# carlosnatalino/optical-rl-gym

Measured on AMD Instinct MI355X. Metric: env-steps/sec RMSA-v0 NSFNET batch 65536, higher is better.
Workload: dtype u64 bitmaps + f64 statistics

## Files before the change

optical_rl_gym_amd/csrc/orl_device_split.h:

```cpp
#pragma once
#include "orl_device_g8.h"

namespace orl {
namespace sp {

#define ORL_PROF_SLOTS 48
#define ORL_PROF_WAVES 16384
#ifdef ORL_TIMING
struct Prof { long long t; unsigned long long acc[ORL_PROF_SLOTS]; };
static __device__ unsigned long long g_prof[ORL_PROF_WAVES * ORL_PROF_SLOTS];
#define ORL_PROF_BEGIN_() do { for (int k_ = 0; k_ < ORL_PROF_SLOTS; k_++) prof.acc[k_] = 0; prof.t = clock64(); } while (0)
#define ORL_PROF_(k) do { long long n_ = clock64(); prof.acc[k] += (unsigned long long)(n_ - prof.t); prof.t = n_; } while (0)
#define ORL_PROF_END_() do { if ((threadIdx.x & 63) == 0) { const size_t w_ = ((size_t)blockIdx.x * (blockDim.x >> 6) + (threadIdx.x >> 6)) % ORL_PROF_WAVES; \
    unsigned long long* g_ = ::orl::sp::g_prof + w_ * ORL_PROF_SLOTS; \
    for (int k_ = 0; k_ < ORL_PROF_SLOTS; k_++) g_[k_] += prof.acc[k_]; } } while (0)
#define ORL_PROF_BEGIN() ORL_PROF_BEGIN_()
#define ORL_PROF_END() ORL_PROF_END_()
#define ORL_PROFA(k) ORL_PROF_(k)
#define ORL_PROF(k) ORL_PROF_(16 + (k))
#define ORL_PROFR(k) ORL_PROF_(32 + (k))
#else
struct Prof { long long t; };
#define ORL_PROF_BEGIN() do { } while (0)
#define ORL_PROF_END() do { } while (0)
// ... 1185 lines not shown
      e.ev_cnt -= n_round;
      e.nfree = (nfree0 + n_round < ORL_FREE_SLOTS) ? nfree0 + n_round : ORL_FREE_SLOTS;
      sink.nrel = nrel0 + n_round;
      e.s_br -= (i64)g8_sum(d_br);
      e.s_nh -= (i64)g8_sum(d_nh);
    } else {
      u64 inf0 = 0;
      PathRec rc0 = PathRec();
      if (ci != 0x7fffffff) { inf0 = (ci == pushed_idx) ? pushed_info : ((ci == pre_idx) ? pre_info : e.ev_info[ci]); rc0 = path_rec_load(P, (int)(inf0 & 0xffffffu)); }
      ORL_PROF(6);
      for (;;) {
        double bt = ct;
        int bi = ci, bl = gl;
  #define ORL_MIN_STEP(CTRL) { double ot = dpp_d<CTRL>(bt); int oi = dpp_i<CTRL>(bi); int ol = dpp_i<CTRL>(bl); \
                               if (ot < bt || (ot == bt && oi < bi)) { bt = ot; bi = oi; bl = ol; } }
        ORL_MIN_STEP(ORL_DPP_XOR1) ORL_MIN_STEP(ORL_DPP_XOR2) ORL_MIN_STEP(ORL_DPP_HALF_MIRROR)
  #undef ORL_MIN_STEP
        if (!(bt <= e.now)) break;
        const u64 info = gget(inf0, bl, lane);
        PathRec rec;
        rec.q[0] = gget(rc0.q[0], bl, lane); rec.q[1] = gget(rc0.q[1], bl, lane);
        rec.q[2] = gget(rc0.q[2], bl, lane); rec.q[3] = gget(rc0.q[3], bl, lane);
        if (gl == (bi & 7)) e.ev_time[bi] = INF;
        if (gl == bl) {
          dirty |= 1 << ck;
          ct = INF; ci = 0x7fffffff;
          int nk = 0;
  #pragma unroll
          for (int k = 0; k < NS; k++) {
            if (k == ck) st[k] = INF;
            const bool due = st[k] <= e.now;
            if (due && (st[k] < ct || (st[k] == ct && si[k] < ci))) { ct = st[k]; ci = si[k]; nk = k; }
          }
          ck = nk;
          if (ci != 0x7fffffff) { inf0 = (ci == pushed_idx) ? pushed_info : ((ci == pre_idx) ? pre_info : e.ev_info[ci]); rc0 = path_rec_load(P, (int)(inf0 & 0xffffffu)); }
        }
        const int s0 = (int)((info >> 24) & 0xfffu), n = (int)((info >> 36) & 0xffu);
        const int core = (int)((info >> 44) & 0x1fu), br = (int)((info >> 49) & 0x7fffu);
        e.ev_cnt--;
        g8::free_push(e, gl, bi);
        sink_add(sink, rec, core, s0, n, lane);
        e.s_br -= br;
        e.s_nh -= (i64)n * path_rec_byte(rec, 0);
      }
    }
    ORL_PROF(7);
    if (e.now < e.t_soon) break;
  }
  {
    double m = st[0];
#pragma unroll
    for (int k = 1; k < NS; k++) m = st[k] < m ? st[k] : m;
    const double lm = g8::g8_min(m);
    e.next_rel = lm < e.t_soon ? lm : e.t_soon;
  }
  out.dirty = dirty;
#pragma unroll
  for (int k = 0; k < NS; k++) { out.t[k] = st[k]; out.i[k] = si[k]; }
  ORL_PROF(8);
}

template <int ENV, int W>
__device__ __forceinline__ void rel_serial(const DevParams& P, i64 env, int lane) {
  u64* s = P.scal + env * ORL_SCAL_WORDS;
  if (!((s[SC_ACC] >> 16) & 1ull)) return;
  const int gl = lane & 7;
  if (gl == 0) atomicAdd(P.q_stat, 1u);
  EnvG e;
  g8::env_load(P, e, env);
  if (P.pipeline2) e.rs = e.cs + 2 * P.C;
  g8::release_due<ENV, W>(P, e, lane);
  e.t_soon = -__builtin_inf();
  if (gl == 0) {
    s[SC_ACC] = s[SC_ACC] & ~(1ull << 16);
    s[SC_NEXTREL] = (u64)__double_as_longlong(e.next_rel);
    s[SC_TSOON] = (u64)__double_as_longlong(e.t_soon);
    s[SC_SBR] = (u64)e.s_br;
    s[SC_SNH] = (u64)e.s_nh;
    s[SC_EV] = pack2(e.ev_hwm, e.ev_cnt);
    s[SC_HINT] = pack2(e.nfree, 0);
  }
}

template <int W, bool CACHED = false>
__device__ __forceinline__ void row_stat_lane(const u64 (&a)[W], int S, RowStat& st, int& max_empty, int& edge, u32* cache = nullptr,
                                              u32 touched = 0u, bool update = false) {
  int nu = 0, lo = 1 << 20, hi = 0, free_ = 0, nf = 0, best = 0, c = 0;
  u64 inter[CACHED ? W : 1];
#pragma unroll
  for (int w = 0; w < W; w++) {
    const u64 maskw = word_mask_lo(S - 64 * w);
    const u64 used = ~a[w] & maskw;
    const u64 prev_top = (w == 0) ? 0ull : (a[w - 1] >> 63);
    const u64 carry_u = (w == 0) ? 0ull : (prev_top ^ 1ull);
    nu += __popcll(used & ~((used << 1) | carry_u));
    if (used) {
      const int l = 64 * w + (int)__builtin_ctzll(used);
      lo = l < lo ? l : lo;
      hi = 64 * w + 64 - (int)__builtin_clzll(used);
    }
    free_ += __popcll(a[w]);
    if (CACHED) {
      const u64 na = ~a[w];
      const bool full = na == 0ull;
      const int lead = full ? 64 : (int)__builtin_ctzll(na), trail = full ? 64 : (int)__builtin_clzll(na);
      best = (c + lead) > best ? (c + lead) : best;
      c = full ? c + 64 : trail;
      inter[CACHED ? w : 0] = full ? 0ull : ((a[w] & (a[w] + 1ull)) & (~0ull >> trail));
    } else if (a[w] == ~0ull) {
      c += 64;
      best = c > best ? c : best;
    } else {
      const int lead = (int)__builtin_ctzll(~a[w]);
      const int inner = word_longest_run_flat(a[w]);
      const int cand = (c + lead) > inner ? (c + lead) : inner;
      best = cand > best ? cand : best;
      c = (int)__builtin_clzll(~a[w]);
    }
  }
  if (CACHED) {
    best = c > best ? c : best;
    u32 cw = *cache;
    u32 need = touched;
#pragma unroll
    for (int w = 0; w < W; w++) {
      const int f = (int)((cw >> (6 * w)) & 63u);
      if (!((touched >> w) & 1u)) {
        if (f == 63) need |= 1u << w;
        else best = f > best ? f : best;
      }
    }
    while (need) {
      const int w = (int)__builtin_ctz(need);
      need &= need - 1u;
      u64 x = inter[0];
#pragma unroll
      for (int k = 1; k < (CACHED ? W : 1); k++) x = (w == k) ? inter[k] : x;
      const int f = word_longest_run_flat(x);
      best = f > best ? f : best;
      cw = (cw & ~(63u << (6 * w))) | ((u32)f << (6 * w));
    }
    if (update) *cache = cw;
  }
  const bool two = nu > 1;
  const int fb = two ? nu - 1 : 0;
  max_empty = best;
  const int tw = (S - 1) >> 6, tb = (S - 1) & 63;
  int top_bit = 0;
#pragma unroll
  for (int w = 0; w < W; w++) top_bit = (w == tw) ? (int)((a[w] >> tb) & 1ull) : top_bit;
  edge = (int)(a[0] & 1ull) + top_bit;
  nf = nu - 1 + edge;
  st.nu = nu; st.lo = lo; st.hi = hi; st.occ = two ? hi - lo : 0; st.fb = fb; st.free_ = free_; st.nf = nf;
}

struct RowInc { int free_, nu, lo, hi, me; };
template <int W> __device__ __forceinline__ u64 row_word(const u64 (&a)[W], int w) {
  u64 x = 0ull;
#pragma unroll
  for (int k = 0; k < W; k++) x = (w == k) ? a[k] : x;
  return x;
}
template <int W> __device__ __forceinline__ int row_run_below(const u64 (&a)[W], int p) {
  int len = 0;
  for (int q = p; q > 0; q -= 64) {
    const int wq = q >> 6, b = q & 63;
    const u64 hi = row_word<W>(a, wq), lo = row_word<W>(a, wq - 1);
    const u64 x = (b == 0) ? lo : ((hi << (64 - b)) | (lo >> b));
    const int c = (x == ~0ull) ? 64 : (int)__builtin_clzll(~x);
    len += c;
    if (c < 64) break;
  }
  return len;
}
template <int W> __device__ __forceinline__ int row_run_from(const u64 (&a)[W], int p) {
  int len = 0;
  for (int q = p; q < 64 * W; q += 64) {
    const int wq = q >> 6, b = q & 63;
    const u64 lo = row_word<W>(a, wq), hi = row_word<W>(a, wq + 1);
    const u64 x = (b == 0) ? lo : ((lo >> b) | (hi << (64 - b)));
    const int c = (x == ~0ull) ? 64 : (int)__builtin_ctzll(~x);
    len += c;
    if (c < 64) break;
  }
  return len;
}
template <int W> __device__ __forceinline__ int row_longest_free(const u64 (&a)[W]) {
  int best = 0, c = 0;
#pragma unroll
  for (int w = 0; w < W; w++) {
    if (a[w] == ~0ull) {
      c += 64;
    } else {
      const int lead = (int)__builtin_ctzll(~a[w]), trail = (int)__builtin_clzll(~a[w]);
      const int inner = word_longest_run_flat((a[w] & (a[w] + 1ull)) & (~0ull >> trail));
      const int cand = (c + lead) > inner ? (c + lead) : inner;
      best = cand > best ? cand : best;
      c = trail;
    }
  }
  return c > best ? c : best;
}
template <int W>
__device__ __forceinline__ void row_inc_apply(u64 (&a)[W], int S, int s0, int n, bool prov, RowInc& s) {
  const int l = row_run_below<W>(a, s0), r = row_run_from<W>(a, s0 + n);
  const int joins = ((s0 > 0 && l == 0) ? 1 : 0) + ((s0 + n < S && r == 0) ? 1 : 0);
  const Mask2 mm = mask2(s0, n);
#pragma unroll
  for (int w = 0; w < W; w++) a[w] ^= mask2_word(mm, w);
  if (prov) {
    s.free_ -= n;
    s.nu += 1 - joins;
    s.lo = s0 < s.lo ? s0 : s.lo;
    s.hi = s0 + n > s.hi ? s0 + n : s.hi;
    if (l + n + r == s.me) s.me = row_longest_free<W>(a);
  } else {
    s.free_ += n;
    s.nu -= 1 - joins;
    const int m = l + n + r;
    s.me = m > s.me ? m : s.me;
    if (s.nu == 0) { s.lo = 1 << 20; s.hi = 0; }
    else {
      if (s0 == s.lo) s.lo = s0 + n + r;
      if (s0 + n == s.hi) s.hi = s0 - l;
    }
  }
}

template <int W>
__device__ __forceinline__ u32 row_inner_cache(const u64* row) {
  u32 cw = 0u;
#pragma unroll
  for (int w = 0; w < (W <= 5 ? W : 0); w++) {
    const u64 a = row[w];
    int f = 0;
    if (a != ~0ull) {
      const int lead = (int)__builtin_ctzll(~a), trail = (int)__builtin_clzll(~a);
      f = word_longest_run(a & ~word_range(0, lead) & ~word_range(64 - trail, 64));
    }
    cw |= (u32)f << (6 * w);
  }
  return cw;
}
__device__ __forceinline__ u32 mask_words(int s0, int n) { return (1u << (s0 >> 6)) | (1u << ((s0 + n - 1) >> 6)); }
template <int W>
__device__ __forceinline__ void row_occ_fb(const u64 (&a)[W], int S, int& occ, int& fb) {
  int nu = 0, lo = 1 << 20, hi = 0;
#pragma unroll
  for (int w = 0; w < W; w++) {
    const u64 used = ~a[w] & word_mask_lo(S - 64 * w);
    const u64 carry_u = (w == 0) ? 0ull : ((a[w > 0 ? w - 1 : 0] >> 63) ^ 1ull);
    nu += __popcll(used & ~((used << 1) | carry_u));
    if (used) {
      const int l = 64 * w + (int)__builtin_ctzll(used);
      lo = l < lo ? l : lo;
      hi = 64 * w + 64 - (int)__builtin_clzll(used);
    }
  }
  const bool two = nu > 1;
  occ = two ? hi - lo : 0;
  fb = two ? nu - 1 : 0;
}

template <int ENV, int W, bool EARLY = false>
__device__ __forceinline__ void row_item_lane1(const DevParams& P, const Wmem& M, const i64 env, const int link, const u32 bits,
                                               const unsigned short* mtab, int second, Prof& prof, bool early_ls = false,
                                               double* stash_env = nullptr, u32* sig = nullptr, u32 sig_val = 0u) {
  const int E = P.E, S = P.S;
  const int nmask = __popc(bits);
  const bool prov_first = (bits & 1u) != 0;
  const bool shared = prov_first && nmask >= 2;
  const bool role_b = shared && second;
  const bool role_a = shared && !second;
  u64* row = wm_bm(P, M, env) + (size_t)link * W;
  int* cs = wm_cs(P, M, env);
  int* rs = cs + 2;
  double* ls = wm_ls(P, M, env) + 4 * link;
  const double now = M.clk ? M.clk[2 * (env - M.clk_env0) + 1] : __longlong_as_double((i64)wm_scal(P, M, env)[SC_NOW]);
  const double now_prov = M.clk ? M.clk[2 * (env - M.clk_env0)] : __longlong_as_double((i64)wm_scal(P, M, env)[SC_NOWA]);
  double2 ls01 = make_double2(0.0, 0.0), ls23 = make_double2(0.0, 0.0);
  if (early_ls && !role_b) { ls01 = *(const double2*)ls; ls23 = *(const double2*)(ls + 2); }
  u32* ocg = (ENV != ENV_RWA && !M.oc0 && M.ocg) ? M.ocg + (env - M.cenv0) * E + link : nullptr;
  u32 ocg_v = 0u;
  if (ocg && !role_b) ocg_v = *ocg;
  u64 a[W];
#pragma unroll
  for (int w = 0; w < W; w++) a[w] = row[w];
  ORL_PROFR(3);
  u64 fin[EARLY ? W : 1];
  u32 later_e = 0u, mw0_e = 0u, mwf_e = 0u;
  if constexpr (EARLY) {
    u32 rest_e = bits & (bits - 1u);
    int first_e = (int)__builtin_ctz(bits);
    if (role_b) { first_e = (int)__builtin_ctz(rest_e); rest_e &= rest_e - 1u; }
    if (role_a) rest_e = 0u;
#pragma unroll
    for (int w = 0; w < W; w++) fin[w] = a[w];
    for (u32 r = bits & ~1u; r; r &= r - 1u) {
      const int k = (int)__builtin_ctz(r);
      const u32 mw = mtab[k];
      const int s0 = (int)(mw & 0x1ff), n = (int)(mw >> 9);
      if (k == first_e) mwf_e = mw;
      if ((rest_e >> k) & 1u) later_e |= mask_words(s0, n);
      const Mask2 mm = mask2(s0, n);
#pragma unroll
      for (int w = 0; w < W; w++) a[w] &= ~mask2_word(mm, w);
    }
    if (bits & 1u) {
      mw0_e = mtab[0];
      if (first_e == 0) mwf_e = mw0_e;
      const Mask2 mm = mask2((int)(mw0_e & 0x1ff), (int)(mw0_e >> 9));
#pragma unroll
      for (int w = 0; w < W; w++) a[w] |= mask2_word(mm, w);
    }
    rw_release_lds();
    if (sig) __hip_atomic_store(sig, sig_val, __ATOMIC_RELAXED, __HIP_MEMORY_SCOPE_WORKGROUP);
    ORL_PROFR(9);
  }
  u32 rest = bits & (bits - 1u);
  int first = (int)__builtin_ctz(bits);
  u32 touched = 0u;
  if (role_b) {
    const u32 mw = EARLY ? mw0_e : (u32)mtab[0];
    const int s0 = (int)(mw & 0x1ff), n = (int)(mw >> 9);
    touched = mask_words(s0, n);
    const Mask2 mm = mask2(s0, n);
#pragma unroll
    for (int w = 0; w < W; w++) a[w] &= ~mask2_word(mm, w);
    first = (int)__builtin_ctz(rest);
    rest &= rest - 1u;
  }
  if (role_a) rest = 0u;
  u32* ocw = (ENV != ENV_RWA && M.oc0) ? M.oc0 + (env - M.cenv0) * E + link : nullptr;
  int occ0 = 0, fb0 = 0;
  if (ENV != ENV_RWA) {
    if (ocg) { }
    else if (!ocw) row_occ_fb<W>(a, S, occ0, fb0);
    else if (!role_b) { const u32 c = *ocw; occ0 = (int)(c >> 16); fb0 = (int)(c & 0xffffu); }
  }
  const bool rel_f = first != 0;
  {
    const u32 mw = EARLY ? mwf_e : (u32)mtab[first];
    const int s0 = (int)(mw & 0x1ff), n = (int)(mw >> 9);
    touched |= mask_words(s0, n);
    const Mask2 mm = mask2(s0, n);
#pragma unroll
    for (int w = 0; w < W; w++) {
      const u64 m = mask2_word(mm, w);
      a[w] = rel_f ? (a[w] | m) : (a[w] & ~m);
    }
  }
  ORL_PROFR(4);
  RowStat after;
  int max_empty = 0, edge = 0;
  u32* icw = (ENV != ENV_RWA && M.ic0) ? M.ic0 + (env - M.cenv0) * E + link : nullptr;
  if (ENV != ENV_RWA) {
#ifdef ORL_DIAG_INSTEAD_OF_ROW_SUMMARY
    ORL_DIAG_INSTEAD_OF_ROW_SUMMARY
#else
    if (W >= 3 && W <= 5 && icw) row_stat_lane<W, (W >= 3 && W <= 5)>(a, S, after, max_empty, edge, icw, touched, !role_a);
    else row_stat_lane<W>(a, S, after, max_empty, edge);
#endif
  } else {
    int f = 0;
#pragma unroll
    for (int w = 0; w < W; w++) f += __popcll(a[w]);
    after.free_ = f;
  }
  ORL_PROFR(5);
  const int free_ = after.free_;
  const double cur_util = div_pos((double)(S - free_), (double)S);
  double cur_frag = 0.0, cur_comp = 0.0;
  if (ENV != ENV_RWA && free_ > 0) {
    int me = (after.nf > 1 && !(after.nf == 2 && edge == 2)) ? max_empty : 0;
    cur_frag = 1.0 - div_pos((double)me, (double)free_);
    if (after.nu > 1) cur_comp = div_pos((double)(after.hi - after.lo), (double)(S - free_)) * div_pos(1.0, (double)after.nu);
    else cur_comp = 1.0;
  }
  if (ocw && role_a) *ocw = ((u32)after.occ << 16) | (u32)after.fb;
  const double clock = rel_f ? now : now_prov;
  const int n_rest = __popc(rest);
#ifdef ORL_DIAG_NO_SECOND_ROUND
  const u64 any_b = 0ull;
#else
  const u64 any_b = __ballot(role_b);
#endif
  for (int round = 0; round < 2; round++) {
    if (round == 1 && !any_b) break;
    if ((round == 1) == role_b) {
      if (role_b || !early_ls) { ls01 = *(const double2*)ls; ls23 = *(const double2*)(ls + 2); }
      double last_update = ls23.y;
      double util = ls01.x, frag = ls01.y, comp = ls23.x;
      if (stash_env && rel_f) { stash_env[2 * link] = util; stash_env[2 * link + 1] = comp; }
#ifdef ORL_DIAG_NO_F64
      if (false) {
#else
      if (clock > 0) {
#endif
        const double time_diff = clock - last_update;
        const Recip rc = recip_of(clock);
        util = div_by((util * last_update) + (cur_util * time_diff), rc);
        if (ENV != ENV_RWA) {
          frag = div_by((frag * last_update) + (cur_frag * time_diff), rc);
          comp = div_by((comp * last_update) + (cur_comp * time_diff), rc);
        }
      }
      last_update = clock;
      if (now > 0 && n_rest > 0) {
        const Recip rn = recip_of(now);
        for (int k = 0; k < n_rest; k++) {
          util = div_by((util * now) + 0.0, rn);
          if (ENV != ENV_RWA) { frag = div_by((frag * now) + 0.0, rn); comp = div_by((comp * now) + 0.0, rn); }
        }
      }
      *(double2*)ls = make_double2(util, frag);
      *(double2*)(ls + 2) = make_double2(comp, last_update);
    }
    wave_fence();
  }
  ORL_PROFR(6);
  if (ocw && role_b) { const u32 c = *ocw; occ0 = (int)(c >> 16); fb0 = (int)(c & 0xffffu); }
  int occL = after.occ, fbL = after.fb;
  if (rest) {
    u32 later = 0u;
    if constexpr (EARLY) {
      later = later_e;
#pragma unroll
      for (int w = 0; w < W; w++) a[w] = fin[w];
    } else {
      for (u32 r = rest; r; r &= r - 1u) {
        const u32 mw = mtab[__builtin_ctz(r)];
        const int s0 = (int)(mw & 0x1ff), n = (int)(mw >> 9);
        later |= mask_words(s0, n);
        const Mask2 mm = mask2(s0, n);
#pragma unroll
        for (int w = 0; w < W; w++) a[w] |= mask2_word(mm, w);
      }
    }
    if (ENV != ENV_RWA) row_occ_fb<W>(a, S, occL, fbL);
    if (icw) {
      u32 cw = *icw;
#pragma unroll
      for (int w = 0; w < (W <= 5 ? W : 0); w++) cw |= ((later >> w) & 1u) ? (63u << (6 * w)) : 0u;
      *icw = cw;
    }
  }
  if (ENV != ENV_RWA) {
    if (ocg) { occ0 = (int)(ocg_v >> 16); fb0 = (int)(ocg_v & 0xffffu); }
    if (ocg && shared) {
      if (role_a) { atomicAdd(cs, -occ0); atomicAdd(cs + 1, -fb0); atomicAdd(rs, -after.occ); atomicAdd(rs + 1, -after.fb); }
      else { atomicAdd(cs, occL); atomicAdd(cs + 1, fbL); atomicAdd(rs, occL); atomicAdd(rs + 1, fbL); }
    } else {
      const int d_occ = occL - occ0, d_fb = fbL - fb0;
      if (d_occ) atomicAdd(cs, d_occ);
      if (d_fb) atomicAdd(cs + 1, d_fb);
      if (rel_f) {
        if (d_occ) atomicAdd(rs, d_occ);
        if (d_fb) atomicAdd(rs + 1, d_fb);
      }
    }
  }
  if (!role_a) {
    if constexpr (!EARLY) {
#pragma unroll
      for (int w = 0; w < W; w++) row[w] = a[w];
    }
    if (ocw) *ocw = ((u32)occL << 16) | (u32)fbL;
    if (ocg) *ocg = ((u32)occL << 16) | (u32)fbL;
  }
  ORL_PROFR(7);
}

template <int ENV, int W>
__device__ __forceinline__ void row_item_lane(const DevParams& P, const Wmem& M, const Item it, Prof& prof) {
  constexpr bool MIXED = true;
  const int E = P.E, S = P.S;
  const i64 env = (i64)(u32)it.a.x;
  const int link = (int)((it.a.x >> 32) & 0xff), nmask = (int)((it.a.x >> 40) & 15);
  const bool release = ((it.a.x >> 44) & 1) != 0;
  const bool prov_first = MIXED && ((it.a.x >> 45) & 1) != 0;
  const u64 cores = it.b.y;
  u64* bm = wm_bm(P, M, env);
  int* cs = wm_cs(P, M, env);
  int* rs = MIXED ? cs + 2 * P.C : nullptr;
  double* ls = wm_ls(P, M, env);
  const double now = M.clk ? M.clk[2 * (env - M.clk_env0) + 1] : __longlong_as_double((i64)wm_scal(P, M, env)[SC_NOW]);
  const double now_prov = M.clk ? M.clk[2 * (env - M.clk_env0)] : __longlong_as_double((i64)wm_scal(P, M, env)[SC_NOWA]);
  const double2 ls01 = *(const double2*)(ls + 4 * link), ls23 = *(const double2*)(ls + 4 * link + 2);
  double last_update = ls23.y;
  double util = ls01.x, frag = ls01.y, comp = ls23.x;
  ORL_PROFR(3);
  u64 a[W];
  int pk = 0, prev_core = -1;
  for (int k = 0; k < nmask; k++) {
    const int core = (int)((cores >> (5 * k)) & 0x1f);
    const u64 mw = k < 4 ? (it.a.y >> (16 * k)) : (it.b.x >> (16 * (k - 4)));
    const int s0 = (int)(mw & 0x1ff), n = (int)((mw >> 9) & 0x7f);
    const bool rel_k = MIXED ? !(k == 0 && prov_first) : release;
    const double clock = (MIXED && !rel_k) ? now_prov : now;
    const bool first_at_clock = (k == 0) || (MIXED && k == 1 && prov_first);
    u64* row = bm + (size_t)(core * E + link) * W;
    if (core != prev_core) {
#pragma unroll
      for (int w = 0; w < W; w++) a[w] = row[w];
      if (ENV != ENV_RWA) {
        int occ_b, fb_b;
        row_occ_fb<W>(a, S, occ_b, fb_b);
        pk = (occ_b << 16) | fb_b;
      }
      prev_core = core;
    }
    {
      const Mask2 mm = mask2(s0, n);
#pragma unroll
      for (int w = 0; w < W; w++) {
        const u64 m = mask2_word(mm, w);
        a[w] = rel_k ? (a[w] | m) : (a[w] & ~m);
        if (m) row[w] = a[w];
      }
    }
    RowStat after;
    int max_empty = 0, edge = 0;
    ORL_PROFR(4);
    if (ENV != ENV_RWA) {
      row_stat_lane<W>(a, S, after, max_empty, edge);
      ORL_PROFR(5);
      const int d_occ = after.occ - (pk >> 16), d_fb = after.fb - (pk & 0xffff);
      pk = (after.occ << 16) | after.fb;
      if (d_occ) atomicAdd(cs + 2 * core, d_occ);
      if (d_fb) atomicAdd(cs + 2 * core + 1, d_fb);
      if (MIXED && rel_k) {
        if (d_occ) atomicAdd(rs + 2 * core, d_occ);
        if (d_fb) atomicAdd(rs + 2 * core + 1, d_fb);
      }
    } else {
      int f = 0;
#pragma unroll
      for (int w = 0; w < W; w++) f += __popcll(a[w]);
      after.free_ = f;
    }
    if (clock > 0) {
      if (first_at_clock) {
        const double time_diff = clock - last_update;
        const int free_ = after.free_;
        const Recip rc = recip_of(clock);
// ... 30 lines not shown
```

optical_rl_gym_amd/csrc/orl_kernels.hip:

```cpp
#include <hip/hip_runtime.h>
#include <stdio.h>
#include <stdlib.h>
#include <algorithm>
#include <vector>

#include "orl_host.h"
#include "orl_persist_form.h"
#include "orl_device_g8.h"
#include "orl_device_split.h"

#ifndef ORL_W
#error "compile with -DORL_W=1|2|5|8"
#endif

using namespace orl;

extern __shared__ __attribute__((aligned(16))) unsigned char orl_lds_raw[];

template <int ENV, int W>
__global__ void __launch_bounds__(64) k_reset(DevParams P, int full, const unsigned char* mask) {
  const i64 env = blockIdx.x;
  const int lane = lane_id();
  if (mask && !mask[env]) return;
  if (lane < 8) P.svc_cnt[(env >> 3) * 64 + (env & 7) * 8 + lane] = 0;
// ... 783 lines not shown
    const u32 listed = (u32)__builtin_amdgcn_readfirstlane((int)rw_load(sync + 0));
    if (asked1 > drawn1 || (listed <= k && asked0 > drawn0)) {
      {
        const int ch = (asked1 > drawn1) ? 1 : 0;
        u32* chan = sync + 4 + 4 * ch;
        sp::rw_acquire_lds();
        const int n_want = __builtin_amdgcn_readfirstlane((int)rw_load(chan + 2));
        const u32 groups = (u32)__builtin_amdgcn_readfirstlane((int)rw_load(chan + 3));
        double* stg_q = (double*)((char*)(sync + ORL_RW_SYNC_WORDS) + ch * (ORL_RW_STAGE_BYTES / 2));
        double* stg_ht = stg_q + 64;
        u32* stg_pk = (u32*)(stg_ht + 64);
        int* stg_cnt = (int*)(stg_pk + 64);
        const i64 env = env0 + (lane >> 3);
        const bool active = env < P.B && ((groups >> (lane >> 3)) & 1u) != 0u;
        sp::SvcBuf sb;
        sb.q = 0.0; sb.ht = 0.0; sb.pk = 0u; sb.cnt = 0;
        sp::svc_generate<ENV>(P, sp::wm_scal(P, M, active ? env : M.scenv0), P.mt + (active ? env : 0) * 624, (P.rates ? P.rates + env0 : nullptr), lane, n_want, sb, active);
        stg_q[lane] = sb.q; stg_ht[lane] = sb.ht; stg_pk[lane] = sb.pk; stg_cnt[lane] = sb.cnt;
        if (ch) drawn1++; else drawn0++;
        rw_signal(chan + 1, ch ? drawn1 : drawn0, lane);
        ORL_PROFR(11);
        continue;
      }
    }
    if (listed <= k) {
      if (gone) break;
      __builtin_amdgcn_s_sleep(2);
      continue;
    }
    sp::rw_acquire_lds();
    ORL_PROFR(8);
    k++;
    sp::sink_compact(s_tab, P.E, lane, s_list, s_list_n);
    wave_fence();
    const int n_items = __builtin_amdgcn_readfirstlane((int)*s_list_n);
    for (int base = 0; base < n_items; base += 64) {
      const int idx = base + lane;
      if (idx < n_items) {
        const int code = (int)s_list[idx];
        const int el = (code >> 8) & 7, link = code & 0xff, second = code >> 15;
        sp::row_item_lane1<ENV, W, true>(P, M, env0 + el, link, s_tab[P.E * el + link].bits, s_mtab + ORL_MTAB * el, second, prof, true, nullptr,
                                         (base + 64 >= n_items) ? sync + 1 : nullptr, k);
      }
    }
    if (n_items == 0) rw_signal(sync + 1, k, lane);
    rw_signal(sync + 2, k, lane);
    ORL_PROFR(10);
  }
  ORL_PROF_END();
}

#ifdef ORL_TIMING
static __device__ unsigned long long g_wts[16384 * 8];
#endif
__device__ __forceinline__ void wave_prio_rotate(int slot, int shift) {
  const int p = (slot + (int)(wall_clock64() >> shift)) & 3;
  if (p == 0) __builtin_amdgcn_s_setprio(0);
  else if (p == 1) __builtin_amdgcn_s_setprio(1);
  else if (p == 2) __builtin_amdgcn_s_setprio(2);
  else __builtin_amdgcn_s_setprio(3);
}
template <int ENV, int W, int LDS_, bool PF, bool RW = false>
__device__ __forceinline__ void persist_body(const DevParams& P, int pol, int target, int* wg_step, u32* n_unfinished) {
  constexpr bool RD = persist_rd_of(LDS_);
  constexpr int LDS = persist_state_of(LDS_);
  constexpr bool CP = PersistCompact<ENV>::value;
  static_assert(!RD || (CP && !RW), "rows deferred: single-core families, one wavefront per 8 envs");
  static_assert(!RW || (CP && (LDS == 1 || LDS == 3)), "two-wavefront form: single-core families, slot maps in LDS");
#ifdef ORL_DIAG_WAVE_SYNC
#define ORL_SYNC() do { wave_fence(); __builtin_amdgcn_wave_barrier(); } while (0)
#else
#define ORL_SYNC() do { if constexpr (RW) { wave_fence(); __builtin_amdgcn_wave_barrier(); } else __syncthreads(); } while (0)
#endif
  constexpr bool SVC = ORL_PERSIST_SVC != 0;
  constexpr bool DS = PersistDeferred<ENV, LDS>::value;
#ifdef ORL_DIAG_NO_MINI
  constexpr bool MINI = false;
#else
  constexpr bool MINI = DS && (LDS == 0 || LDS == 3);
#endif
  const int ICL = (PersistInner<ENV, W, LDS>::value && !RD) ? P.persist_ic : 0;
  const bool IC = ICL >= 1, OC = ICL >= 2;
  constexpr bool SR = PF;
  const PersistLds L = persist_lds_layout(P.E, P.H, P.bm_words, P.C, LDS, CP, ICL, PersistDeferred<ENV, 0>::value, RD);
  typename sp::SinkEntryOf<CP>::type* s_tab = (typename sp::SinkEntryOf<CP>::type*)(orl_lds_raw + L.tab);
  u32* s_tally = (u32*)(orl_lds_raw + L.tally);
  unsigned short* s_mtab = (unsigned short*)(orl_lds_raw + L.mtab);
  unsigned short* s_list = (unsigned short*)(orl_lds_raw + L.list);
  int* s_deferred = (int*)(orl_lds_raw + L.misc);
  u32* s_list_n = (u32*)(orl_lds_raw + L.misc + 8);
  u32* rw_sync = (u32*)(orl_lds_raw + L.total);
  sp::CtrlLds<CP> T = {s_tab, s_tally, L.tw, s_mtab, s_list, s_list_n, s_deferred, rw_sync};
  u32 rw_asked0 = 0u, rw_asked1 = 0u;
  u32 rw_early = 0u, rw_early_groups = 0u;
#define ORL_RW_TAKE(AREA, LANE)                                                                                           \
  do {                                                                                                                   \
    const double* q_ = (const double*)((const char*)(rw_sync + ORL_RW_SYNC_WORDS) + (AREA) * (ORL_RW_STAGE_BYTES / 2));    \
    svb.q = q_[LANE]; svb.ht = q_[64 + (LANE)]; svb.pk = ((const u32*)(q_ + 128))[LANE]; svb.cnt = ((const int*)(q_ + 128))[64 + (LANE)]; \
  } while (0)
#define ORL_RW_ASK(AREA, BALLOT, NWANT, LANE)                                                                             \
  do {                                                                                                                   \
    u32 groups_ = 0u;                                                                                                    \
    for (int g_ = 0; g_ < 8; g_++) groups_ |= (u32)(((BALLOT) >> (8 * g_)) & 1ull) << g_;                               \
    if ((LANE) == 0) { rw_sync[6 + 4 * (AREA)] = (u32)(NWANT); rw_sync[7 + 4 * (AREA)] = groups_; }                       \
    if ((AREA) == 0) { rw_asked0++; rw_early = rw_asked0; rw_early_groups = groups_; }                                   \
    else rw_asked1++;                                                                                                    \
    rw_signal(rw_sync + 4 + 4 * (AREA), (AREA) ? rw_asked1 : rw_asked0, (LANE));                                         \
  } while (0)
  if constexpr (RW) {
    if (threadIdx.x < ORL_RW_SYNC_WORDS) rw_sync[threadIdx.x] = 0u;
    __syncthreads();
    if (threadIdx.x >= 64) {
      persist_row_wave<ENV, W, LDS>(P, L, ICL, rw_sync);
      return;
    }
  }
  const int lane = lane_id();
  const i64 env0 = (i64)blockIdx.x * 8;
  const i64 env = env0 + (threadIdx.x >> 3);
  const int nenv = (int)(P.B - env0 < 8 ? P.B - env0 : 8);
  int step = wg_step[blockIdx.x];
  const int fair = RW ? 0 : P.persist_fair;
  const int wslot = (int)__builtin_amdgcn_s_getreg(4 | (0 << 6) | (3 << 11));
  sp::Prof prof;
#ifdef ORL_TIMING
  unsigned long long wts0 = wall_clock64(), wts1 = 0, wts2 = 0;
#endif
  const bool pend = (env < P.B) && ((P.scal[env * ORL_SCAL_WORDS + SC_ACC] >> 16) & 1ull) != 0ull;
  const bool valid = env < P.B;
  sp::SoonRegs soon_c;
  soon_c.dirty = 0;
  sp::SvcBuf svb;
  svb.q = 0.0; svb.ht = 0.0; svb.pk = 0u; svb.cnt = 0;
  sp::StepCarry C;
  C.soon = SR ? &soon_c : nullptr;
  C.svc = SVC ? &svb : nullptr;
  u64 now0_w = 0ull;
#define ORL_LOAD_CARRIED()                                                                                  \
  do {                                                                                                      \
    C.desc = valid ? P.svc_desc[env] : 0ull;                                                                \
    if (DS && valid && step < target) {                                                                     \
      C.esp = (int)P.scal[env * ORL_SCAL_WORDS + SC_ESP];                                                   \
      if (ENV == ENV_RMCSA) {   \
        const u64 acc_ = P.scal[env * ORL_SCAL_WORDS + SC_ACC];                                             \
        C.prev_core = (acc_ & 2ull) ? (int)((acc_ >> 32) & 31ull) : 0;                                      \
      }                                                                                                     \
      now0_w = P.scal[env * ORL_SCAL_WORDS + SC_NOW];                                                       \
    }                                                                                                       \
    if (SVC && valid && step < target) {                                                                    \
      const size_t sl_ = (size_t)blockIdx.x * 64 + (size_t)lane;                                            \
      svb.cnt = P.svc_cnt[sl_];                                                                             \
      if (!sp::svc_empty(svb)) { svb.q = P.svc_q[sl_]; svb.ht = P.svc_ht[sl_]; svb.pk = P.svc_pk[sl_]; }   \
    }                                                                                                       \
    _Pragma("unroll") for (int k = 0; k < ORL_SOON_PER_LANE; k++) {                                         \
      const bool ld = SR && valid && step < target;                                                         \
      soon_c.t[k] = ld ? P.soon_t[env * ORL_SOON + (lane & 7) + 8 * k] : __builtin_inf();                   \
      soon_c.i[k] = ld ? (int)P.soon_i[env * ORL_SOON + (lane & 7) + 8 * k] : 0;                            \
    }                                                                                                       \
  } while (0)
  sp::Wmem M = sp::wmem_global(P);
  constexpr bool REC = (LDS == 1 || LDS == 2);
  if (LDS != 2 && !RD) {
    M.clk = (double*)(orl_lds_raw + L.clk);
    M.clk_env0 = env0;
  }
  if (LDS >= 1) {
// ... 158 lines not shown
          if (rw_early != 0u && __ballot(want && early_mine) != 0ull) {
            rw_wait(rw_sync + 5, rw_early);
            if (want && early_mine) { ORL_RW_TAKE(0, lane_i); want = false; }
            rw_early = 0u;
            rw_early_groups = 0u;
          }
          if (__ballot(want) != 0ull) {
            ORL_RW_ASK(1, __ballot(want), (left < 8 ? left : 8), lane_i);
            rw_wait(rw_sync + 9, rw_asked1);
            if (want) ORL_RW_TAKE(1, lane_i);
          }
          wave_fence();
        } else {
          sp::svc_generate<ENV>(P, sp::wm_scal(P, M, valid_i ? env_i : M.scenv0), P.mt + (valid_i ? env_i : 0) * 624, (P.rates ? P.rates + env0 : nullptr), lane_i, left < 8 ? left : 8, svb, need);
        }
      }
#endif
    }
    ORL_PROFA(0);
    sp::CtrlOpts O;
    O.persistent = true;
    O.write_io = (step + 1 == target);
    O.trusted = true;
    O.emit_queue = false;
    O.prefetch = PF;
    O.auto_reset = true;
    O.rank_pairs = SR;
    O.parity = 0;
    int done_i = 0;
    {
      int a[4];
      ScanHand hand;
      hand.n = 1; hand.q[0] = hand.q[1] = hand.q[2] = hand.q[3] = 0ull;
      hand.words = (P.H + 2 + 7) >> 3;
#ifdef ORL_DIAG_INSTEAD_OF_SCAN
      constexpr bool HAND = false;
      int pop_pre = -2;
      ORL_DIAG_INSTEAD_OF_SCAN
#else
      constexpr bool HAND = DS && ENV != ENV_RMCSA;
      int pop_pre = -2;
      if (HAND) {
        pop_pre = -1;
        if (valid_i) {
          u64* rec_i = sp::wm_scal(P, M, env_i);
          const int nfree = (int)(u32)*sp::mrec<MINI>(M, rec_i, env_i, SC_HINT);
          if (nfree > 0) pop_pre = (int)((const unsigned short*)(rec_i + SC_FREE0))[nfree - 1];
        }
      }
      policy_g<ENV, W, 8>(P, sp::wm_bm(P, M, valid_i ? env_i : M.env0), valid_i, (int)(u32)C.desc, (int)((C.desc >> 32) & 0xffffu),
                          (int)((C.desc >> 48) & 0xffu), lane_i, pol, (pol == POL_PATH_FF && valid_i) ? P.path_col[env_i] : 0, a,
                          HAND ? &hand : nullptr);
#endif
      const int4 av = make_int4(a[0], a[1], a[2], a[3]);
      ORL_PROFA(1);
      if (fair) wave_prio_rotate(wslot, fair);
      T.deferred = &s_deferred[step & 1];
      C.t = step - first_step;
      sp::ctrl_phase<ENV, W, CP, DS, MINI, DS && RW, DS && RD>(P, M, O, T, C, env_i, valid_i, lane_i, prof, &av, &done_i, nullptr,
                                                               HAND ? &hand : nullptr, pop_pre);
    }
    ORL_SYNC();
    if (fair) wave_prio_rotate(wslot, fair);
    if constexpr (RW) {
      C.rw_k++;
      rw_signal(rw_sync + 0, C.rw_k, lane_i);
      if constexpr (SVC) {
        const bool one_left = valid_i && ((svb.cnt & 0xff) + 1 == (svb.cnt >> 8));
        const int lim = DS ? first_step + P.log_cap : target;
        const int after = target - step - 2;
        if (s_deferred[step & 1] == 0 && step + 1 < (lim < target ? lim : target) && after >= 1 && rw_early == 0u) {
          const u64 bw = __ballot(one_left);
          if (bw != 0ull) ORL_RW_ASK(0, bw, (after < 8 ? after : 8), lane_i);
        }
      }
      ORL_PROFA(12);
    } else if constexpr (!RD) {
#ifdef ORL_DIAG_NO_ROWS
      const int n_items = 0;
#else
      const int n_items = (int)*s_list_n;
#endif
      ORL_PROFA(12);
      for (int idx = lane_i; idx < n_items; idx += 64) {
        const int code = (int)s_list[idx];
        const int el = (code >> 8) & 7, link = code & 0xff, second = code >> 15;
        if constexpr (!CP) {
          if (!second) sp::row_item_lane<ENV, W>(P, M, sp::item_from_sink(env0 + el, link, s_tab[P.E * el + link]), prof);
        } else {
          sp::row_item_lane1<ENV, W>(P, M, env0 + el, link, s_tab[P.E * el + link].bits, s_mtab + ORL_MTAB * el, second, prof, PF);
        }
      }
      ORL_PROFA(13);
    }
    const bool deferred = s_deferred[step & 1] != 0;
    if (ENV == ENV_DEEPRMSA && (O.write_io || deferred)) {
      ORL_SYNC();
      if (valid_i) {
        if (MINI) {
          u64 sd, br;
          sp::svc_words<ENV>(P, C.desc, sd, br);
          obs8_env_w<W>(P, sp::wm_bm(P, M, env_i), sd, br, env_i, lane_i, done_i);
        } else {
          obs8_env<W>(P, sp::wm_bm(P, M, env_i), sp::wm_scal(P, M, env_i), env_i, lane_i, done_i);
        }
      }
    }
    step++;
    if (deferred) { left_pending = true; break; }
    if constexpr (RD) { if (__ballot(valid_i && C.ecur + 1 + P.rel_limit > P.elog_cap) != 0ull) break; }
  }
  ORL_PROF_END();
#ifdef ORL_TIMING
  wts2 = wall_clock64();
#endif
  if constexpr (RW) {
    rw_wait(rw_sync + 2, C.rw_k);
    if (SVC && rw_early != 0u) {
      rw_wait(rw_sync + 5, rw_early);
      if (valid && ((rw_early_groups >> (lane >> 3)) & 1u) != 0u) ORL_RW_TAKE(0, lane);
    }
    rw_signal(rw_sync + 3, 1u, lane);
  }
  const bool finished_run = P.persist_finish && step > first_step && !left_pending;
  if (DS) {
    if (step > first_step) {
      ORL_SYNC();
      int tid_t = (int)threadIdx.x;
      asm volatile("" : "+v"(tid_t));
      const i64 env_t = env0 + (tid_t >> 3);
      if (ENV != ENV_RWA && !RD && env_t < P.B && (tid_t & 7) == 0) {
        int* cs = sp::wm_cs(P, M, env_t);
        int* rs = cs + 2 * P.C;
        const int pc = (ENV == ENV_RMCSA) ? C.prev_core : 0;
        int occ, fb;
        if (!M.cs_lds) { occ = atomicAdd(cs + 2 * pc, 0) - atomicAdd(rs + 2 * pc, 0); fb = atomicAdd(cs + 2 * pc + 1, 0) - atomicAdd(rs + 2 * pc + 1, 0); }
        else { occ = cs[2 * pc] - rs[2 * pc]; fb = cs[2 * pc + 1] - rs[2 * pc + 1]; }
        P.slog[(size_t)(3 * (step - first_step) + 1) * (size_t)P.log_stride + (size_t)env_t] = sp::slog_w1(false, 0, 0, occ, fb);
      }
    }
    if (threadIdx.x == 0) P.log_n[blockIdx.x] = (step - first_step) | (finished_run ? (1 << 16) : 0);
    if constexpr (RD) {
      int tid_e = (int)threadIdx.x;
      asm volatile("" : "+v"(tid_e));
      const i64 env_e = env0 + (tid_e >> 3);
      if (env_e < P.B && (tid_e & 7) == 0) P.elog_n[env_e] = C.ecur;
    }
  } else if (PersistDeferred<ENV, 0>::value && threadIdx.x == 0) {
    P.log_n[blockIdx.x] = 0;
  }
  if (P.persist_finish && step > first_step && !left_pending) {
    ORL_SYNC();
    u32 f = 0u;
    int tid_f = (int)threadIdx.x;
    asm volatile("" : "+v"(tid_f));
    const i64 env_f = env0 + (tid_f >> 3);
    if (env_f < P.B && (tid_f & 7) == 0) {
      u64* s = sp::wm_scal(P, M, env_f);
      int* cs = sp::wm_cs(P, M, env_f);
      int* rs = cs + 2 * P.C;
      const u64 acc = DS ? 0ull : s[SC_ACC];
      if ((u32)acc & 2u) {
        const int c0 = (int)((acc >> 32) & 31);
        const i64 s_nh_prov = (i64)(acc >> 37);
        int occ, fb;
        if (!M.cs_lds) {
// ... 825 lines not shown
```

Before: 1.526 billion.

## Use idle wavefront lanes to help busy lanes with row work

Per-link row items are processed one per lane, so the last partial batch of 64 leaves many lanes idle. This change recruits those idle lanes in two ways. First, a lane whose item has several later masks hands the occupancy and fragmentation recomputation to an idle lane. Second, inside the cached row summary, a second stale word's longest-run computation is sent to an idle lane through ds_permute/bpermute. The cost is extra ballots, cross-lane permutes, a new role encoding, and more per-link statistic atomics, which add overhead and correctness risk.

```diff
diff --git a/optical_rl_gym_amd/csrc/orl_device_split.h b/optical_rl_gym_amd/csrc/orl_device_split.h
--- a/optical_rl_gym_amd/csrc/orl_device_split.h
+++ b/optical_rl_gym_amd/csrc/orl_device_split.h
@@ -1291,9 +1291,11 @@
   }
 }
 
-template <int W, bool CACHED = false>
+template <int W, bool CACHED = false, bool HELP = false>
 __device__ __forceinline__ void row_stat_lane(const u64 (&a)[W], int S, RowStat& st, int& max_empty, int& edge, u32* cache = nullptr,
-                                              u32 touched = 0u, bool update = false) {
+                                              u32 touched = 0u, bool update = false, int* diag = nullptr, bool idle = false,
+                                              int n_live = 64) {
+  static_assert(!HELP || CACHED, "the second-word hand-off belongs to the cached summary");
   int nu = 0, lo = 1 << 20, hi = 0, free_ = 0, nf = 0, best = 0, c = 0;
   u64 inter[CACHED ? W : 1];
 #pragma unroll
@@ -1339,6 +1341,56 @@
         else best = f > best ? f : best;
       }
     }
+#ifdef ORL_TIMING
+    if (diag) { diag[0] = __popc(need); diag[1] = 0; }
+#endif
+    if constexpr (HELP) {
+      if (idle) need = 0u;
+      const bool has1 = need != 0u;
+      const int w1 = has1 ? (int)__builtin_ctz(need) : 0;
+      need &= need - 1u;
+      u64 x = inter[0];
+#pragma unroll
+      for (int k = 1; k < (CACHED ? W : 1); k++) x = (w1 == k) ? inter[k] : x;
+      const bool want = need != 0u;
+      const u64 bw = __ballot(want);
+      const bool handoff = bw != 0ull && n_live < 64;
+      const int w2 = want ? (int)__builtin_ctz(need) : 0;
+      const int me = lane_id();
+      int peer = me;
+      bool served = false;
+      if (handoff) {
+        const int h = n_live + (int)__builtin_amdgcn_mbcnt_hi((u32)(bw >> 32), __builtin_amdgcn_mbcnt_lo((u32)bw, 0u));
+        served = want && h < 64;
+        peer = served ? h : me;
+        u64 x2 = inter[0];
+#pragma unroll
+        for (int k = 1; k < (CACHED ? W : 1); k++) x2 = (w2 == k) ? inter[k] : x2;
+        const int dst = (served ? h : (idle ? 0 : me)) << 2;
+        const u32 r_lo = (u32)__builtin_amdgcn_ds_permute(dst, (int)(u32)x2);
+        const u32 r_hi = (u32)__builtin_amdgcn_ds_permute(dst, (int)(u32)(x2 >> 32));
+        if (idle) x = ((u64)r_hi << 32) | (u64)r_lo;
+#ifdef ORL_TIMING
+        if (diag) diag[1] = 1;
+#endif
+      }
+      const int f = word_longest_run_flat(x);
+      if (has1) {
+        best = f > best ? f : best;
+        cw = (cw & ~(63u << (6 * w1))) | ((u32)f << (6 * w1));
+      }
+      if (handoff) {
+        const int f2 = __builtin_amdgcn_ds_bpermute(peer << 2, f);
+        if (served) {
+          best = f2 > best ? f2 : best;
+          cw = (cw & ~(63u << (6 * w2))) | ((u32)f2 << (6 * w2));
+          need &= need - 1u;
+        }
+      }
+    }
+#ifdef ORL_TIMING
+    if (diag) diag[2] = need != 0u ? 1 : 0;
+#endif
     while (need) {
       const int w = (int)__builtin_ctz(need);
       need &= need - 1u;
@@ -1471,16 +1523,21 @@
   fb = two ? nu - 1 : 0;
 }
 
-template <int ENV, int W, bool EARLY = false>
+template <int ENV, int W, bool EARLY = false, bool HELP = false>
 __device__ __forceinline__ void row_item_lane1(const DevParams& P, const Wmem& M, const i64 env, const int link, const u32 bits,
                                                const unsigned short* mtab, int second, Prof& prof, bool early_ls = false,
-                                               double* stash_env = nullptr, u32* sig = nullptr, u32 sig_val = 0u) {
+                                               double* stash_env = nullptr, u32* sig = nullptr, u32 sig_val = 0u, int n_live = 64) {
+  static_assert(!HELP || (!EARLY && ENV != ENV_RWA), "helper lanes: RMSA / DeepRMSA in the one-wavefront forms");
   const int E = P.E, S = P.S;
   const int nmask = __popc(bits);
   const bool prov_first = (bits & 1u) != 0;
+  const bool idle = HELP && (second & 8) != 0;
+  const bool role_c = HELP && (second & 2) != 0;
+  const bool has_c = HELP && (second & 1) != 0;
+  const bool nostat = role_c || idle;
   const bool shared = prov_first && nmask >= 2;
-  const bool role_b = shared && second;
-  const bool role_a = shared && !second;
+  const bool role_b = shared && (HELP ? (second & 4) != 0 : second != 0);
+  const bool role_a = shared && !role_b && !role_c;
   u64* row = wm_bm(P, M, env) + (size_t)link * W;
   int* cs = wm_cs(P, M, env);
   int* rs = cs + 2;
@@ -1488,10 +1545,10 @@
   const double now = M.clk ? M.clk[2 * (env - M.clk_env0) + 1] : __longlong_as_double((i64)wm_scal(P, M, env)[SC_NOW]);
   const double now_prov = M.clk ? M.clk[2 * (env - M.clk_env0)] : __longlong_as_double((i64)wm_scal(P, M, env)[SC_NOWA]);
   double2 ls01 = make_double2(0.0, 0.0), ls23 = make_double2(0.0, 0.0);
-  if (early_ls && !role_b) { ls01 = *(const double2*)ls; ls23 = *(const double2*)(ls + 2); }
+  if (early_ls && !role_b && !nostat) { ls01 = *(const double2*)ls; ls23 = *(const double2*)(ls + 2); }
   u32* ocg = (ENV != ENV_RWA && !M.oc0 && M.ocg) ? M.ocg + (env - M.cenv0) * E + link : nullptr;
   u32 ocg_v = 0u;
-  if (ocg && !role_b) ocg_v = *ocg;
+  if (ocg && !role_b && !nostat) ocg_v = *ocg;
   u64 a[W];
 #pragma unroll
   for (int w = 0; w < W; w++) a[w] = row[w];
@@ -1527,7 +1584,7 @@
     ORL_PROFR(9);
   }
   u32 rest = bits & (bits - 1u);
-  int first = (int)__builtin_ctz(bits);
+  int first = idle ? 0 : (int)__builtin_ctz(bits);
   u32 touched = 0u;
   if (role_b) {
     const u32 mw = EARLY ? mw0_e : (u32)mtab[0];
@@ -1549,7 +1606,7 @@
   }
   const bool rel_f = first != 0;
   {
-    const u32 mw = EARLY ? mwf_e : (u32)mtab[first];
+    const u32 mw = EARLY ? mwf_e : (idle ? (1u << 9) : (u32)mtab[first]);
     const int s0 = (int)(mw & 0x1ff), n = (int)(mw >> 9);
     touched |= mask_words(s0, n);
     const Mask2 mm = mask2(s0, n);
@@ -1557,6 +1614,19 @@
     for (int w = 0; w < W; w++) {
       const u64 m = mask2_word(mm, w);
       a[w] = rel_f ? (a[w] | m) : (a[w] & ~m);
+    }
+  }
+  if constexpr (HELP) {
+    if (role_c) {
+      for (u32 r = rest; r; r &= r - 1u) {
+        const u32 mw = mtab[__builtin_ctz(r)];
+        const int s0 = (int)(mw & 0x1ff), n = (int)(mw >> 9);
+        touched |= mask_words(s0, n);
+        const Mask2 mm = mask2(s0, n);
+#pragma unroll
+        for (int w = 0; w < W; w++) a[w] |= mask2_word(mm, w);
+      }
+      rest = 0u;
     }
   }
   ORL_PROFR(4);
@@ -1567,8 +1637,21 @@
 #ifdef ORL_DIAG_INSTEAD_OF_ROW_SUMMARY
     ORL_DIAG_INSTEAD_OF_ROW_SUMMARY
 #else
-    if (W >= 3 && W <= 5 && icw) row_stat_lane<W, (W >= 3 && W <= 5)>(a, S, after, max_empty, edge, icw, touched, !role_a);
+    int diag[3] = {0, 0, 0};
+    if (W >= 3 && W <= 5 && icw)
+      row_stat_lane<W, (W >= 3 && W <= 5), HELP && (W >= 3 && W <= 5)>(a, S, after, max_empty, edge, icw, touched, !role_a && !has_c && !idle,
+                                                                       diag, idle, n_live);
     else row_stat_lane<W>(a, S, after, max_empty, edge);
+#ifdef ORL_TIMING
+    if constexpr (!EARLY) {
+      int mx = 0;
+      for (int r = 1; r <= 6; r++) mx = (__ballot(!idle && diag[0] >= r) != 0ull) ? r : mx;
+      prof.acc[42] += 1ull; prof.acc[43] += (unsigned long long)mx; prof.acc[44] += mx >= 2 ? 1ull : 0ull;
+      prof.acc[45] += (__ballot(rest != 0u || role_c) != 0ull) ? 1ull : 0ull;
+      prof.acc[46] += (__ballot(diag[1] != 0) != 0ull) ? 1ull : 0ull;
+      prof.acc[47] += (__ballot(diag[2] != 0) != 0ull) ? 1ull : 0ull;
+    }
+#endif
 #endif
   } else {
     int f = 0;
@@ -1596,7 +1679,7 @@
 #endif
   for (int round = 0; round < 2; round++) {
     if (round == 1 && !any_b) break;
-    if ((round == 1) == role_b) {
+    if ((round == 1) == role_b && !nostat) {
       if (role_b || !early_ls) { ls01 = *(const double2*)ls; ls23 = *(const double2*)(ls + 2); }
       double last_update = ls23.y;
       double util = ls01.x, frag = ls01.y, comp = ls23.x;
@@ -1630,7 +1713,7 @@
   ORL_PROFR(6);
   if (ocw && role_b) { const u32 c = *ocw; occ0 = (int)(c >> 16); fb0 = (int)(c & 0xffffu); }
   int occL = after.occ, fbL = after.fb;
-  if (rest) {
+  if (rest && !has_c) {
     u32 later = 0u;
     if constexpr (EARLY) {
       later = later_e;
@@ -1656,7 +1739,11 @@
   }
   if (ENV != ENV_RWA) {
     if (ocg) { occ0 = (int)(ocg_v >> 16); fb0 = (int)(ocg_v & 0xffffu); }
-    if (ocg && shared) {
+    if (HELP && (has_c || role_c)) {
+      if (role_c) { atomicAdd(cs, occL); atomicAdd(cs + 1, fbL); atomicAdd(rs, occL); atomicAdd(rs + 1, fbL); }
+      else if (!(ocg && shared)) { atomicAdd(cs, -occ0); atomicAdd(cs + 1, -fb0); atomicAdd(rs, -occ0); atomicAdd(rs + 1, -fb0); }
+    } else if (HELP && idle) {
+    } else if (ocg && shared) {
       if (role_a) { atomicAdd(cs, -occ0); atomicAdd(cs + 1, -fb0); atomicAdd(rs, -after.occ); atomicAdd(rs + 1, -after.fb); }
       else { atomicAdd(cs, occL); atomicAdd(cs + 1, fbL); atomicAdd(rs, occL); atomicAdd(rs + 1, fbL); }
     } else {
@@ -1669,7 +1756,7 @@
       }
     }
   }
-  if (!role_a) {
+  if (!role_a && !has_c && !idle) {
     if constexpr (!EARLY) {
 #pragma unroll
       for (int w = 0; w < W; w++) row[w] = a[w];
diff --git a/optical_rl_gym_amd/csrc/orl_kernels.hip b/optical_rl_gym_amd/csrc/orl_kernels.hip
--- a/optical_rl_gym_amd/csrc/orl_kernels.hip
+++ b/optical_rl_gym_amd/csrc/orl_kernels.hip
@@ -889,6 +889,11 @@
   const int ICL = (PersistInner<ENV, W, LDS>::value && !RD) ? P.persist_ic : 0;
   const bool IC = ICL >= 1, OC = ICL >= 2;
   constexpr bool SR = PF;
+#ifdef ORL_DIAG_NO_ROW_HELP
+  constexpr bool HELP = false;
+#else
+  constexpr bool HELP = CP && PersistInner<ENV, W, LDS>::value && !RW && !RD;
+#endif
   const PersistLds L = persist_lds_layout(P.E, P.H, P.bm_words, P.C, LDS, CP, ICL, PersistDeferred<ENV, 0>::value, RD);
   typename sp::SinkEntryOf<CP>::type* s_tab = (typename sp::SinkEntryOf<CP>::type*)(orl_lds_raw + L.tab);
   u32* s_tally = (u32*)(orl_lds_raw + L.tally);
@@ -1213,6 +1218,36 @@
       const int n_items = (int)*s_list_n;
 #endif
       ORL_PROFA(12);
+      if constexpr (HELP) {
+        const int n_all = __builtin_amdgcn_readfirstlane(n_items);
+        for (int base = 0; base < n_all; base += 64) {
+          const int idx = base + lane_i;
+          bool idle = idx >= n_all;
+          int code = idle ? 0 : (int)s_list[idx];
+          u32 bits = idle ? 0u : s_tab[P.E * ((code >> 8) & 7) + (code & 0xff)].bits;
+          int role = (code >> 15) << 2;
+          int n_live = n_all - base;
+          const bool want_c = __popc(bits >> 1) >= 2 && ((bits & 1u) == 0u || role != 0);
+          const u64 bc = __ballot(want_c);
+          if (bc != 0ull && n_live < 64) {
+            const int h = n_live + (int)__builtin_amdgcn_mbcnt_hi((u32)(bc >> 32), __builtin_amdgcn_mbcnt_lo((u32)bc, 0u));
+            const bool served = want_c && h < 64;
+            const int got = __builtin_amdgcn_ds_permute((served ? h : (idle ? 0 : lane_i)) << 2, code);
+            role |= served ? 1 : 0;
+            const int n_c = (int)__popcll(bc);
+            if (idle && lane_i < n_live + n_c) {
+              code = got & 0x7fff;
+              bits = s_tab[P.E * ((code >> 8) & 7) + (code & 0xff)].bits;
+              role = 2;
+              idle = false;
+            }
+            n_live = n_live + n_c < 64 ? n_live + n_c : 64;
+          }
+          const int el = (code >> 8) & 7, link = code & 0xff;
+          sp::row_item_lane1<ENV, W, false, true>(P, M, env0 + el, link, bits, s_mtab + ORL_MTAB * el, idle ? 8 : role, prof, PF, nullptr, nullptr,
+                                                  0u, n_live);
+        }
+      } else
       for (int idx = lane_i; idx < n_items; idx += 64) {
         const int code = (int)s_list[idx];
         const int el = (code >> 8) & 7, link = code & 0xff, second = code >> 15;
```

Result: no change. 1.544 billion, median of 6 (+1.2%).
